# kamenbliznashki/chexpert

Hardware: AMD Instinct MI355X
Metric: images/sec fwd+bwd DenseNet121 320x320 bf16 (per-GPU rate in config.images_per_sec_per_gpu) (higher is better)
Workload: dtype bf16; 1 GPU; densenet121 bf16 1xMI355X 320x320 bs=256 per GPU, U-Ones labels (BASELINE configs[1]); 14 classes; random-init weights, synthetic uint8 X-rays; per_gpu_batch=256, global_batch=256, parallelism=dp1, rccl_ranks=1, capture_failed=0, launch=hipGraph replay

## Files before the change

chexpert_amd/csrc/common.h:

```cpp
#pragma once
#include <hip/hip_runtime.h>
#include <stdint.h>
#include <stdio.h>
#include "../../include/chexpert_hip.h"

#ifdef CX_DIAG
#include <stdlib.h>
static inline int cx_diag_int(const char* name, int dflt) {
  const char* e = getenv(name);
  return e ? atoi(e) : dflt;
}
static inline bool cx_diag_set(const char* name) { return getenv(name) != nullptr; }
#else
static inline int cx_diag_int(const char*, int dflt) { return dflt; }
static inline bool cx_diag_set(const char*) { return false; }
#endif

typedef __bf16 bf16;
typedef __attribute__((ext_vector_type(8))) __bf16 bf16x8;
typedef __attribute__((ext_vector_type(4))) __bf16 bf16x4;
typedef __attribute__((ext_vector_type(4))) short s16x4;
typedef __attribute__((ext_vector_type(16))) float f32x16;
typedef __attribute__((ext_vector_type(4))) float f32x4;

// ... 245 lines not shown
extern thread_local int cx_tl_slab_floats_v;
static inline float* dw_slab(float* scratch, long long scratch_floats, long long splits, long long total) {
  const bool ok = scratch && splits * total <= scratch_floats && splits * total < (1ll << 31);
  cx_tl_slab_floats_v = ok ? (int)(splits * total) : 0;
  return ok ? scratch : nullptr;
}
int cx_dw_reduce(float* dw, const float* slab, size_t total, int splits, hipStream_t st);
int cx_dw_reduce_ld(float* dw, const float* slab, size_t total, int splits, int cols, int dw_ld, hipStream_t st);

static inline int stat_rows_check(const CxConv& p, int rows) {
  if (!p.stat_det || !p.stat_sum) return 0;
  if (rows > p.stat_replicas || p.stat_rstride < p.N) return CX_ESTATROWS;
  cx_tl_stat_rows = rows;
  return 0;
}
```

chexpert_amd/csrc/conv1x1_bwd.hip:

```cpp
#include <cstdlib>
#include <type_traits>
#include "common.h"

namespace {

#ifndef CX_PW_NT
#define CX_PW_NT 7
#endif
constexpr int PW_NT = CX_PW_NT;
constexpr int KD = 128;
constexpr int BM = 128;
constexpr int PITCH = KD * 2 + 16;
constexpr int A_BYTES = BM * PITCH;
constexpr int XH_PITCH = 64;
constexpr int XH_BYTES = BM * XH_PITCH;

template <int CTRL>
__device__ __forceinline__ float dpp_add(float v) {
  return v + __int_as_float(__builtin_amdgcn_update_dpp(0, __float_as_int(v), CTRL, 0xF, 0xF, true));
}
__device__ __forceinline__ float half_sum(float v) {
  v = dpp_add<0xB1>(v);
  v = dpp_add<0x4E>(v);
  v = dpp_add<0x141>(v);
// ... 219 lines not shown
    wg_stat_end<NT / 64>(scratch, BC, tid, NT, p.stat_sum, p.stat_sq, p.stat_det, p.stat_det ? split : (int)blockIdx.x, p.stat_replicas,
                         p.stat_rstride, c0, p.N);
  }
}

constexpr int BM2 = 64;
#ifdef CX_PW_FWD_ORDER
#define TILE_OF(mt) (mt)
#else
#define TILE_OF(mt) (m_tiles - 1 - (mt))
#endif
constexpr int A2_BYTES = BM2 * PITCH;
constexpr int XH2_BYTES = BM2 * XH_PITCH;
typedef uint32_t pw_u32x4 __attribute__((ext_vector_type(4)));
__device__ __forceinline__ uint4 as_u4(const pw_u32x4 v) { return make_uint4(v[0], v[1], v[2], v[3]); }

template <int PRO, bool ACC>
__global__ __launch_bounds__(512, 1) void pw_bwd2_kernel(const CxConv p, float* __restrict__ dw, const int M, const int c_tiles,
                                                         const int tiles_per_split, float* __restrict__ slab, const int dw_ld) {
  constexpr int BC = 128, NT = 512;
  constexpr int W_BYTES = BC * PITCH;
  constexpr int COEF_BYTES = (5 * BC + 3 * KD) * 4;
  extern __shared__ __attribute__((aligned(16))) char smem[];
  float* ecoef = reinterpret_cast<float*>(smem);
  char* Wt = smem + COEF_BYTES;
  char* At = Wt + W_BYTES;
  char* Xh = At + 2 * A2_BYTES;
  char* Xt = Xh + 2 * 4 * XH2_BYTES;
  char* Ot = Xt + A2_BYTES;

  const int tid = threadIdx.x, lane = tid & 63, wave = tid >> 6;
  const int lrow = lane & 31, lh = lane >> 5;
  const int id = xcd_remap(blockIdx.x, gridDim.x);
  const int ct = id % c_tiles, split = id / c_tiles;
  const int c0 = ct * BC;
  const int m_tiles = (M + BM2 - 1) / BM2;
  const int t0 = split * tiles_per_split;
  const int t1 = (t0 + tiles_per_split < m_tiles) ? t0 + tiles_per_split : m_tiles;

  const bf16* __restrict__ X = reinterpret_cast<const bf16*>(p.x);
  const bf16* __restrict__ X2 = reinterpret_cast<const bf16*>(p.x2);
  const bf16* __restrict__ Wp = reinterpret_cast<const bf16*>(p.w);
  const bf16* __restrict__ EX = reinterpret_cast<const bf16*>(p.ex);
  bf16* __restrict__ Y = reinterpret_cast<bf16*>(p.y);

  if (tid < BC) {
    const int n = c0 + tid;
    const bool ok = n < p.N;
    ecoef[tid] = ok ? p.e_sc[n] : 0.f;
    ecoef[BC + tid] = ok ? p.e_sh[n] : 0.f;
    ecoef[2 * BC + tid] = ok ? p.e_mu[n] : 0.f;
    ecoef[3 * BC + tid] = ok ? p.e_r[n] : 0.f;
    ecoef[4 * BC + tid] = ok ? p.e_scale[n] : 0.f;
  }
  const int q = tid & 15, r0 = tid >> 4;
#pragma unroll
  for (int i = 0; i < BC / 32; ++i) {
    const int n = c0 + r0 + 32 * i;
    const uint4 v = *reinterpret_cast<const uint4*>(Wp + (size_t)(n < p.N ? n : 0) * KD + q * 8);
    *reinterpret_cast<uint4*>(Wt + (r0 + 32 * i) * PITCH + q * 16) = n < p.N ? v : make_uint4(0, 0, 0, 0);
  }
  if (PRO == CX_PRO_AFFINE2 && tid < KD) {
    ecoef[5 * BC + tid] = p.pa[tid];
    ecoef[5 * BC + KD + tid] = p.pb[tid];
    ecoef[5 * BC + 2 * KD + tid] = p.pc[tid];
  }
  const float* aco = ecoef + 5 * BC + q * 8;

  const int pw = wave & 1, cq = wave >> 1;
  const int wn = wave & 3, wc0 = (wave >> 2) * 2;
  f32x16 accw[2];
#pragma unroll
  for (int i = 0; i < 2; ++i)
#pragma unroll
    for (int r = 0; r < 16; ++r) accw[i][r] = 0.f;
  float s1[2][8], s2[2][8];
#pragma unroll
  for (int cc = 0; cc < 2; ++cc)
#pragma unroll
    for (int e = 0; e < 8; ++e) s1[cc][e] = s2[cc][e] = 0.f;

// ... 14 lines not shown
        else os[i] = *reinterpret_cast<const pw_u32x4*>(Y + (size_t)mmc * p.ldy + qcl);
      } else os[i] = pw_u32x4{0u, 0u, 0u, 0u};
    }
  };
  auto request_dz = [&](int mt) __attribute__((always_inline)) {
#pragma unroll
    for (int i = 0; i < 2; ++i) {
      const int mm = TILE_OF(mt) * BM2 + r0 + 32 * i;
      const int mmc = mm < M ? mm : M - 1;
      ru[i] = *reinterpret_cast<const pw_u32x4*>(X + (size_t)mmc * p.ldx + q * 8);
      if (PRO == CX_PRO_AFFINE2) rv[i] = *reinterpret_cast<const pw_u32x4*>(X2 + (size_t)mmc * p.ldx2 + q * 8);
    }
  };
  request_dz(t0);
  request_rmw(t0, xsA, osA);
  request_rmw(t0 + 1 < t1 ? t0 + 1 : t0, xsB, osB);
  __syncthreads();

  auto tile = [&](const int mt, auto SelC, pw_u32x4 (&xs)[2], pw_u32x4 (&os)[2]) __attribute__((always_inline)) {
    constexpr int SEL = decltype(SelC)::value;
    const int m0 = TILE_OF(mt) * BM2;
    const bool tvalid = mt < t1;
    char* Ab_ = At + SEL * A2_BYTES;
    char* Xb_ = Xh + SEL * (4 * XH2_BYTES);
    char* Ob_ = Ot + SEL * A2_BYTES;
#pragma unroll
    for (int i = 0; i < 2; ++i) {
      const int row = r0 + 32 * i;
      U128 o;
      if (PRO == CX_PRO_NONE) o.u = as_u4(ru[i]);
      else o.u = cx_affine2_8(as_u4(ru[i]), as_u4(rv[i]), aco, aco + KD, aco + 2 * KD);
      const unsigned keep = (tvalid && m0 + row < M) ? 0xffffffffu : 0u;
      o.u.x &= keep; o.u.y &= keep; o.u.z &= keep; o.u.w &= keep;
      *reinterpret_cast<uint4*>(Ab_ + row * PITCH + q * 16) = o.u;
      *reinterpret_cast<pw_u32x4*>(Xt + row * PITCH + q * 16) = xs[i];
      *reinterpret_cast<pw_u32x4*>(Ob_ + row * PITCH + q * 16) = os[i];
    }
    __syncthreads();
    request_dz(mt + 1 < t1 ? mt + 1 : t1 - 1);
    f32x16 accd;
#pragma unroll
    for (int r = 0; r < 16; ++r) accd[r] = 0.f;
    {
      const char* Ab = Ab_ + (pw * 32 + lrow) * PITCH + lh * 16;
      const char* Wb = Wt + (cq * 32 + lrow) * PITCH + lh * 16;
#pragma unroll
      for (int kk = 0; kk < KD / 16; ++kk) {
        const bf16x8 af = *reinterpret_cast<const bf16x8*>(Ab + kk * 32);
        const bf16x8 wf = *reinterpret_cast<const bf16x8*>(Wb + kk * 32);
        accd = __builtin_amdgcn_mfma_f32_32x32x16_bf16(wf, af, accd, 0, 0, 0);
      }
    }
    const int m = m0 + pw * 32 + lrow;
    const bool pok = tvalid && m < M;
#pragma unroll
    for (int cc = 0; cc < 2; ++cc) {
      const int cl = cq * 32 + 8 * (2 * cc + lh);
// ... 33 lines not shown
    for (int kk = 0; kk < BM2 / 16; ++kk) {
      const bf16x8 af = tr_frag(Ab_, PITCH, kk * 16, wn * 32, lane);
#pragma unroll
      for (int i = 0; i < 2; ++i) {
        const bf16x8 bfr = tr_frag(Xb_ + (wc0 + i) * XH2_BYTES, XH_PITCH, kk * 16, 0, lane);
        accw[i] = __builtin_amdgcn_mfma_f32_32x32x16_bf16(af, bfr, accw[i], 0, 0, 0);
      }
    }
  };

  const int n_pairs = (t1 - t0 + 1) >> 1;
  for (int pr_ = 0; pr_ < n_pairs; ++pr_) {
    tile(t0 + 2 * pr_, std::integral_constant<int, 0>{}, xsA, osA);
    tile(t0 + 2 * pr_ + 1, std::integral_constant<int, 1>{}, xsB, osB);
  }

#pragma unroll
  for (int i = 0; i < 2; ++i) {
    const int c = c0 + (wc0 + i) * 32 + lrow;
    if (c < p.N) {
#pragma unroll
      for (int r = 0; r < 16; ++r) {
        const int n = wn * 32 + (r & 3) + 8 * (r >> 2) + 4 * lh;
        dw_out(dw, slab, (size_t)KD * p.N, split, slab ? (size_t)n * p.N + c : (size_t)n * dw_ld + c, accw[i][r]);
      }
    }
  }
  {
    __syncthreads();
    float* scratch = reinterpret_cast<float*>(At);
    wg_stat_begin<8>(scratch, BC, tid, NT);
    float t1v = 0.f, t2v = 0.f;
#pragma unroll
    for (int cc = 0; cc < 2; ++cc)
#pragma unroll
      for (int e = 0; e < 8; ++e) {
        const float a = half_sum(s1[cc][e]);
        const float b = half_sum(s2[cc][e]);
        if (lrow == 8 * cc + e) { t1v = a; t2v = b; }
      }
    if (lrow < 16) {
      const int cl = cq * 32 + 8 * (2 * (lrow >> 3) + lh) + (lrow & 7);
      wg_stat_put(scratch, BC, wave, cl, t1v, ecoef[3 * BC + cl] * (t2v - ecoef[2 * BC + cl] * t1v));
    }
    wg_stat_end<8>(scratch, BC, tid, NT, p.stat_sum, p.stat_sq, p.stat_det, p.stat_det ? split : (int)blockIdx.x, p.stat_replicas,
                   p.stat_rstride, c0, p.N);
  }
}

struct PairLayer {
  const bf16* x;
  const bf16* x2;
  const bf16* w;
  const float *pa, *pb, *pc;
  const float *e_sc, *e_sh, *e_mu, *e_r, *e_scale;
  float *stat_sum, *stat_sq;
  float* dw;
  float* slab;
  int ldx, ldx2, dw_ld, stat_rstride;
};

template <bool ACC>
// ... 403 lines not shown
  if (const int e = pair_check(*pa)) return e;
  if (const int e = pair_check(*pb)) return e;
  const CxConv &a = *pa, &b = *pb;
  if (a.ex != b.ex || a.y != b.y || a.N != b.N || a.B != b.B || a.H != b.H || a.W != b.W || a.ldex != b.ldex || a.ldy != b.ldy ||
      a.accumulate != b.accumulate || a.stat_det != b.stat_det || a.stat_replicas != b.stat_replicas ||
      dw_ld_a < a.N || a.stat_sum == b.stat_sum)
    return CX_EINVAL;
  hipStream_t st = as_stream(stream);
  return a.accumulate ? launch_bwd2p<true>(a, b, dw_a, dw_ld_a, dw_b, scratch, scratch_floats, st)
                      : launch_bwd2p<false>(a, b, dw_a, dw_ld_a, dw_b, scratch, scratch_floats, st);
}

extern "C" int cx_conv1x1_dgrad_wgrad(const CxConv* pp, float* dw, void* stream) {
  return cx_conv1x1_dgrad_wgrad_ws(pp, dw, nullptr, 0, stream);
}
```

chexpert_amd/csrc/conv1x1_fwdk.hip:

```cpp
#include <cstdlib>
#include "common.h"

namespace {

constexpr int BM = 128, BN = 128;
constexpr int WAVES_N = 2, TM = 2, TN = 2;
constexpr int EPITCH = BN + 4;

template <int BK, int PRO>
__global__ __launch_bounds__(256, 2) void pw_fwdk_kernel(const CxConv p, const int M) {
  constexpr int PITCH = BK * 2 + 16;
  constexpr int CPR = BK / 8;
  constexpr int RPP = 256 / CPR;
  constexpr int NL = 128 / RPP;
  constexpr int A_BYTES = BM * PITCH;
  extern __shared__ __attribute__((aligned(16))) char smem[];
  float* coef = reinterpret_cast<float*>(smem);
  char* At = smem + 2 * p.K * 4;
  char* Bt = At + A_BYTES;
  const int tid = threadIdx.x, lane = tid & 63, wave = tid >> 6;
  const int wm = wave / WAVES_N, wn = wave % WAVES_N;
  const int mt = xcd_remap(blockIdx.x, gridDim.x);
  const bf16* __restrict__ X = reinterpret_cast<const bf16*>(p.x);
  const bf16* __restrict__ Wp = reinterpret_cast<const bf16*>(p.w);
  bf16* __restrict__ Y = reinterpret_cast<bf16*>(p.y);

  if (PRO == CX_PRO_AFFINE_RELU)
    for (int i = tid; i < p.K; i += 256) { coef[i] = p.pa[i]; coef[p.K + i] = p.pb[i]; }

  const int q = tid % CPR, r0 = tid / CPR;
  const int nsteps = (p.K + BK - 1) / BK;
  uint4 ra[NL], rw[NL];
  bool kok = true;
  auto issue_loads = [&](int s) __attribute__((always_inline)) {
    const int c = s * BK + q * 8;
    kok = c < p.K;
    const int cc = kok ? c : 0;
#pragma unroll
    for (int i = 0; i < NL; ++i) {
      const int row = r0 + RPP * i;
      const int m = mt * BM + row;
      const int mc = m < M ? m : M - 1;
      ra[i] = *reinterpret_cast<const uint4*>(X + (size_t)mc * p.ldx + cc);
// ... 15 lines not shown
      }
      *reinterpret_cast<uint4*>(At + row * PITCH + q * 16) = o.u;
      *reinterpret_cast<uint4*>(Bt + row * PITCH + q * 16) = kok ? rw[i] : make_uint4(0, 0, 0, 0);
    }
  };

  f32x16 acc[TM][TN];
#pragma unroll
  for (int i = 0; i < TM; ++i)
#pragma unroll
    for (int j = 0; j < TN; ++j)
#pragma unroll
      for (int r = 0; r < 16; ++r) acc[i][j][r] = 0.f;

  issue_loads(0);
  __syncthreads();
  const int lrow = lane & 31, lh = lane >> 5;
  for (int s = 0; s < nsteps; ++s) {
    write_stage(s);
    __syncthreads();
    if (s + 1 < nsteps) issue_loads(s + 1);
#pragma unroll
    for (int kk = 0; kk < BK / 16; ++kk) {
      bf16x8 af[TM], bfr[TN];
#pragma unroll
      for (int i = 0; i < TM; ++i) af[i] = *reinterpret_cast<const bf16x8*>(At + ((wm * TM + i) * 32 + lrow) * PITCH + kk * 32 + lh * 16);
#pragma unroll
      for (int j = 0; j < TN; ++j) bfr[j] = *reinterpret_cast<const bf16x8*>(Bt + ((wn * TN + j) * 32 + lrow) * PITCH + kk * 32 + lh * 16);
#pragma unroll
      for (int i = 0; i < TM; ++i)
#pragma unroll
        for (int j = 0; j < TN; ++j) acc[i][j] = __builtin_amdgcn_mfma_f32_32x32x16_bf16(af[i], bfr[j], acc[i][j], 0, 0, 0);
    }
    __syncthreads();
  }

  constexpr int ECPR = BN / 8, ERPP = 256 / ECPR, NPASS = 64 / ERPP;
  const int cq = tid % ECPR, rr = tid / ECPR;
  float* etile = reinterpret_cast<float*>(At);
  float s1[8], s2[8];
#pragma unroll
  for (int j = 0; j < 8; ++j) s1[j] = s2[j] = 0.f;
  const bool want_stats = p.stat_sum != nullptr;
#pragma unroll
  for (int half = 0; half < 2; ++half) {
    if (wm == half) {
#pragma unroll
      for (int i = 0; i < TM; ++i)
#pragma unroll
        for (int j = 0; j < TN; ++j)
#pragma unroll
// ... 20 lines not shown
            w4[j] = cx_packbf(v[2 * j], v[2 * j + 1]);
            const float rl = cx_bf_lo(w4[j]), rh = cx_bf_hi(w4[j]);
            s1[2 * j] += rl;
            s1[2 * j + 1] += rh;
            s2[2 * j] += rl * rl;
            s2[2 * j + 1] += rh * rh;
          }
          o.u = make_uint4(w4[0], w4[1], w4[2], w4[3]);
        }
        *reinterpret_cast<uint4*>(Y + (size_t)m * p.ldy + cq * 8) = o.u;
      }
    }
    __syncthreads();
  }
  if (want_stats) {
#pragma unroll
    for (int j = 0; j < 8; ++j) {
#pragma unroll
      for (int d = ECPR; d < 64; d <<= 1) {
        s1[j] += __shfl_xor(s1[j], d);
        s2[j] += __shfl_xor(s2[j], d);
      }
    }
    float* scratch = reinterpret_cast<float*>(At);
    wg_stat_begin<4>(scratch, BN, tid, 256);
    if (lane < ECPR) {
#pragma unroll
      for (int j = 0; j < 8; ++j) wg_stat_put(scratch, BN, wave, cq * 8 + j, s1[j], s2[j]);
    }
    wg_stat_end<4>(scratch, BN, tid, 256, p.stat_sum, p.stat_sq, p.stat_det, (int)blockIdx.x, p.stat_replicas, p.stat_rstride, 0, p.N);
  }
}

template <int PRO, int D>
__global__ __launch_bounds__(256, 2) void pw_fwdp_kernel(const CxConv p, const int M) {
  constexpr int BK = 64;
  constexpr int PITCH = BK * 2 + 16;
  constexpr int CPR = BK / 8;
  constexpr int RPP = 256 / CPR;
  constexpr int NL = 128 / RPP;
  constexpr int A_BYTES = BM * PITCH;
  extern __shared__ __attribute__((aligned(16))) char smem[];
  float* coef = reinterpret_cast<float*>(smem);
  char* At = smem + 2 * p.K * 4;
  char* Bt = At + A_BYTES;
  const int tid = threadIdx.x, lane = tid & 63, wave = tid >> 6;
  const int wm = wave / WAVES_N, wn = wave % WAVES_N;
  const int mt = xcd_remap(blockIdx.x, gridDim.x);
  const bf16* __restrict__ X = reinterpret_cast<const bf16*>(p.x);
  const bf16* __restrict__ Wp = reinterpret_cast<const bf16*>(p.w);
  bf16* __restrict__ Y = reinterpret_cast<bf16*>(p.y);
  if (PRO == CX_PRO_AFFINE_RELU)
    for (int i = tid; i < p.K; i += 256) { coef[i] = p.pa[i]; coef[p.K + i] = p.pb[i]; }
  const int q = tid % CPR, r0 = tid / CPR;
  const int nsteps = (p.K + BK - 1) / BK;
  const bf16* xr[NL];
  const bf16* wr[NL];
#pragma unroll
  for (int i = 0; i < NL; ++i) {
    const int row = r0 + RPP * i;
    const int m = mt * BM + row;
    xr[i] = X + (size_t)(m < M ? m : M - 1) * p.ldx + q * 8;
    wr[i] = Wp + (size_t)row * p.K + q * 8;
  }
  uint4 ra[D][NL], rw[D][NL];
  auto issue = [&](uint4 (&a)[NL], uint4 (&w)[NL], int s) __attribute__((always_inline)) {
    const int sc = s < nsteps ? s : nsteps - 1;
    int c = sc * BK;
// ... 17 lines not shown
        o.u = a[i];
      } else {
        o.u = cx_affine_relu8(a[i], coef + c0, coef + p.K + c0);
      }
      *reinterpret_cast<uint4*>(At + row * PITCH + q * 16) = o.u;
      *reinterpret_cast<uint4*>(Bt + row * PITCH + q * 16) = kok ? w[i] : make_uint4(0, 0, 0, 0);
    }
  };
  f32x16 acc[TM][TN];
#pragma unroll
  for (int i = 0; i < TM; ++i)
#pragma unroll
    for (int j = 0; j < TN; ++j)
#pragma unroll
      for (int r = 0; r < 16; ++r) acc[i][j][r] = 0.f;
#pragma unroll
  for (int d = 0; d < D; ++d) issue(ra[d], rw[d], d);
  __syncthreads();
  const int lrow = lane & 31, lh = lane >> 5;
  for (int s0 = 0; s0 < nsteps; s0 += D) {
#pragma unroll
    for (int d = 0; d < D; ++d) {
      const int s = s0 + d;
      if (s < nsteps) {
        stage(ra[d], rw[d], s);
        __syncthreads();
        issue(ra[d], rw[d], s + D);
#pragma unroll
        for (int kk = 0; kk < BK / 16; ++kk) {
          bf16x8 af[TM], bfr[TN];
#pragma unroll
          for (int i = 0; i < TM; ++i) af[i] = *reinterpret_cast<const bf16x8*>(At + ((wm * TM + i) * 32 + lrow) * PITCH + kk * 32 + lh * 16);
#pragma unroll
          for (int j = 0; j < TN; ++j) bfr[j] = *reinterpret_cast<const bf16x8*>(Bt + ((wn * TN + j) * 32 + lrow) * PITCH + kk * 32 + lh * 16);
#pragma unroll
          for (int i = 0; i < TM; ++i)
#pragma unroll
            for (int j = 0; j < TN; ++j) acc[i][j] = __builtin_amdgcn_mfma_f32_32x32x16_bf16(af[i], bfr[j], acc[i][j], 0, 0, 0);
        }
        __syncthreads();
      }
    }
  }
  constexpr int ECPR = BN / 8, ERPP = 256 / ECPR, NPASS = 64 / ERPP;
  const int cq = tid % ECPR, rr = tid / ECPR;
  float* etile = reinterpret_cast<float*>(At);
  float s1[8], s2[8];
#pragma unroll
  for (int j = 0; j < 8; ++j) s1[j] = s2[j] = 0.f;
  const bool want_stats = p.stat_sum != nullptr;
#pragma unroll
  for (int half = 0; half < 2; ++half) {
    if (wm == half) {
#pragma unroll
      for (int i = 0; i < TM; ++i)
#pragma unroll
        for (int j = 0; j < TN; ++j)
#pragma unroll
// ... 20 lines not shown
            w4[j] = cx_packbf(v[2 * j], v[2 * j + 1]);
            const float rl = cx_bf_lo(w4[j]), rh = cx_bf_hi(w4[j]);
            s1[2 * j] += rl;
            s1[2 * j + 1] += rh;
            s2[2 * j] += rl * rl;
            s2[2 * j + 1] += rh * rh;
          }
          o.u = make_uint4(w4[0], w4[1], w4[2], w4[3]);
        }
        *reinterpret_cast<uint4*>(Y + (size_t)m * p.ldy + cq * 8) = o.u;
      }
    }
    __syncthreads();
  }
  if (want_stats) {
#pragma unroll
    for (int j = 0; j < 8; ++j) {
#pragma unroll
      for (int d = ECPR; d < 64; d <<= 1) {
        s1[j] += __shfl_xor(s1[j], d);
        s2[j] += __shfl_xor(s2[j], d);
      }
    }
    float* scratch = reinterpret_cast<float*>(At);
    wg_stat_begin<4>(scratch, BN, tid, 256);
    if (lane < ECPR) {
#pragma unroll
      for (int j = 0; j < 8; ++j) wg_stat_put(scratch, BN, wave, cq * 8 + j, s1[j], s2[j]);
    }
    wg_stat_end<4>(scratch, BN, tid, 256, p.stat_sum, p.stat_sq, p.stat_det, (int)blockIdx.x, p.stat_replicas, p.stat_rstride, 0, p.N);
  }
}

template <int PRO, int D>
int launch_fwdp(const CxConv& p, hipStream_t st) {
  const long long M = (long long)p.B * p.Ho * p.Wo;
  const int m_tiles = (int)((M + BM - 1) / BM);
  const size_t stage = (size_t)2 * BM * (64 * 2 + 16);
  const size_t epi = (size_t)64 * EPITCH * 4;
  const size_t smem = (size_t)2 * p.K * 4 + (stage > epi ? stage : epi) + 2 * BN * 4;
  static bool attr = false;
  if (!attr) {
    (void)hipFuncSetAttribute(reinterpret_cast<const void*>(&pw_fwdp_kernel<PRO, D>), hipFuncAttributeMaxDynamicSharedMemorySize, 80 * 1024);
    attr = true;
  }
  if (smem > 80 * 1024) return CX_ESHAPE;
// ... 28 lines not shown
  *handled = false;
  if (p.mode != CX_MODE_CONV || p.kh != 1 || p.kw != 1 || p.stride != 1 || p.pad != 0 || p.tstride > 1) return 0;
  if (p.epilogue != CX_EPI_STORE || p.accumulate || p.N != 128 || p.K <= 256 || p.K > 1280) return 0;
  if (p.prologue != CX_PRO_AFFINE_RELU && p.prologue != CX_PRO_NONE) return 0;
  if ((long long)p.B * p.Ho * p.Wo > 200000) return 0;
  *handled = true;
  static const int pipe = cx_diag_int("CX_FWDK_PIPE", 2);
  if (pipe == 2 && p.K % 32 == 0 && p.K >= 512)
    return p.prologue == CX_PRO_AFFINE_RELU ? launch_fwdp<CX_PRO_AFFINE_RELU, 2>(p, st) : launch_fwdp<CX_PRO_NONE, 2>(p, st);
  if (pipe == 3 && p.K % 32 == 0 && p.K >= 192)
    return p.prologue == CX_PRO_AFFINE_RELU ? launch_fwdp<CX_PRO_AFFINE_RELU, 3>(p, st) : launch_fwdp<CX_PRO_NONE, 3>(p, st);
  if (pipe == 4 && p.K % 32 == 0 && p.K >= 256)
    return p.prologue == CX_PRO_AFFINE_RELU ? launch_fwdp<CX_PRO_AFFINE_RELU, 4>(p, st) : launch_fwdp<CX_PRO_NONE, 4>(p, st);
  return p.prologue == CX_PRO_AFFINE_RELU ? launch_fwdk<128, CX_PRO_AFFINE_RELU>(p, st) : launch_fwdk<128, CX_PRO_NONE>(p, st);
}
```

chexpert_amd/csrc/conv3x3_ring.hip:

```cpp
#include <cstdlib>
#include <type_traits>
#include "common.h"

namespace {

constexpr int XP = 272;
constexpr int NT = 512;
constexpr int W_ROWS = 9 * 32;
constexpr int W_BYTES = W_ROWS * XP;
constexpr int RING_PX_MAX = (160 * 1024 - W_BYTES - 1024 - 256) / XP;

struct RingGeo {
  int B, H, W, P, R, Q;
  int Wt, ntx;
  int spi;
  int steps_per_wg;
  unsigned mP;
  unsigned mSpi;
  int ntx_shift;
};

__device__ __forceinline__ int wrapq(int v, int q) { return v >= q ? v - q : v; }
__device__ __forceinline__ int div_spi(const RingGeo& g, int v) { return g.spi == 1 ? v : (int)__umulhi((unsigned)v, g.mSpi); }

template <int CTRL>
__device__ __forceinline__ float dpp_get(float v) { return __int_as_float(__builtin_amdgcn_update_dpp(0, __float_as_int(v), CTRL, 0xF, 0xF, true)); }
template <int XOR>
__device__ __forceinline__ float swz_xor(float v) { return __int_as_float(__builtin_amdgcn_ds_swizzle(__float_as_int(v), (XOR << 10) | 0x1F)); }
__device__ __forceinline__ float half_sum16(const float (&v)[16], int lane) {
  const bool b0 = lane & 1, b1 = lane & 2, b2 = lane & 4, b3 = lane & 8;
  float a[8], b[4], c[2];
#pragma unroll
  for (int k = 0; k < 8; ++k) a[k] = (b0 ? v[2 * k + 1] : v[2 * k]) + dpp_get<0xB1>(b0 ? v[2 * k] : v[2 * k + 1]);
#pragma unroll
  for (int k = 0; k < 4; ++k) b[k] = (b1 ? a[2 * k + 1] : a[2 * k]) + dpp_get<0x4E>(b1 ? a[2 * k] : a[2 * k + 1]);
#pragma unroll
  for (int k = 0; k < 2; ++k) c[k] = (b2 ? b[2 * k + 1] : b[2 * k]) + swz_xor<4>(b2 ? b[2 * k] : b[2 * k + 1]);
  const float d = (b3 ? c[1] : c[0]) + swz_xor<8>(b3 ? c[0] : c[1]);
  return d + swz_xor<16>(d);
}

#ifdef CX_RING_STAMPS
__device__ unsigned long long ring_stamps[1024 * 8];
__device__ unsigned long long ring_fwd_stamps[1024 * 8];
__device__ __forceinline__ unsigned long long rstamp() {
  unsigned long long t;
  __builtin_amdgcn_sched_barrier(0);
  asm volatile("s_memtime %0\n\ts_waitcnt lgkmcnt(0)" : "=s"(t)::"memory");
  __builtin_amdgcn_sched_barrier(0);
  return t;
}
#define RSTAMP(i) { const unsigned long long t_ = rstamp(); st_acc[i] += t_ - st_prev; st_prev = t_; }
__device__ unsigned long long ring_pro_stamps[1024 * 8];
__device__ unsigned long long ring_fwd_pro_stamps[1024 * 8];
#define PSTAMP_BEGIN unsigned long long ps_acc[3] = {0, 0, 0}; const unsigned long long ps_rt0 = __builtin_amdgcn_s_memrealtime(), ps_t0 = rstamp(); \
  unsigned long long ps_prev = ps_t0; bool ps_first = true;
#define PSTAMP(i) { const unsigned long long t_ = rstamp(); ps_acc[i] = t_ - ps_prev; ps_prev = t_; }
#define PSTAMP_FIRST_MFMA if (ps_first) { PSTAMP(1) ps_first = false; }
#define PSTAMP_MARK ps_prev = rstamp();
#define PSTAMP_END(arr) { PSTAMP(2) const unsigned long long rt_ = __builtin_amdgcn_s_memrealtime(); \
  if (threadIdx.x == 0 && blockIdx.x < 1024) { for (int i = 0; i < 3; ++i) arr[blockIdx.x * 8 + i] = ps_acc[i]; \
    arr[blockIdx.x * 8 + 3] = ps_prev - ps_t0; arr[blockIdx.x * 8 + 4] = rt_ - ps_rt0; } }
#else
#define RSTAMP(i)
#define PSTAMP_BEGIN
#define PSTAMP(i)
#define PSTAMP_FIRST_MFMA
#define PSTAMP_MARK
#define PSTAMP_END(arr)
#endif
template <int NCH, int DEPTH>
__global__ __launch_bounds__(NT, 1) void conv3x3_ring_fwd_kernel(const bf16* __restrict__ x, int ldx, const float* __restrict__ sc,
                                                                const float* __restrict__ sh, const bf16* __restrict__ wpk,
                                                                bf16* __restrict__ y, int ldy, float* stat_sum, float* stat_sq,
                                                                int stat_replicas, int stat_rstride, int stat_det, const RingGeo g) {
  extern __shared__ __attribute__((aligned(16))) char smem[];
  float* coef = reinterpret_cast<float*>(smem);
  char* wl = smem + 1024 + 256;
  char* ring = wl + W_BYTES;
  const int tid = threadIdx.x, lane = tid & 63, wave = tid >> 6;
  const int lrow = lane & 31, lh = lane >> 5;
  const int P = g.P, R = g.R, Q = g.Q, W = g.W, H = g.H, Wt = g.Wt, ntx = g.ntx;
  PSTAMP_BEGIN

// ... 934 lines not shown
```

scratch/trace_step.py:

```python
import csv, re, sys
rows = [r for r in csv.DictReader(open(sys.argv[1]))]
rows.sort(key=lambda r: int(r['Start_Timestamp']))
name = lambda r: re.sub(r'\(.*', '', r['Kernel_Name'].replace('void (anonymous namespace)::', '').replace('(anonymous namespace)::', ''))[:48]
idx = [i for i, r in enumerate(rows) if 'adam' in r['Kernel_Name']]
pairs = [(x, y) for x, y in zip(idx, idx[1:]) if y - x > 200]
which = int(sys.argv[2]) if len(sys.argv) > 2 else len(pairs) // 2
a, b = pairs[which]
step = rows[a + 1:b + 1]
t0 = int(step[0]['Start_Timestamp'])
last_end = t0
print("# %d steps; step %d: %d kernels, %.3f ms" % (len(pairs), which, len(step), (int(step[-1]['End_Timestamp']) - t0) / 1e6))
for r in step:
    s, e = int(r['Start_Timestamp']), int(r['End_Timestamp'])
    print("%9.1f %8.1f %7.1f q%-3s %s  g=%s wg=%s" % ((s - t0) / 1e3, (e - s) / 1e3, (s - last_end) / 1e3, r.get('Queue_Id', '?')[-3:], name(r),
                                                   r.get('Grid_Size', r.get('Grid_Size_X', '?')), r.get('Workgroup_Size', r.get('Workgroup_Size_X', '?'))))
    last_end = max(last_end, e)
```

Baseline: 9665 images/sec.

## Overlap pointwise conv prologue loads and shorten BN-stat wave reductions

In the 1x1 conv forward and backward kernels, the weight tile and BN coefficient loads are now issued into registers alongside the first activation tile loads. They are stored to LDS only after a scheduling barrier, so their global latency overlaps instead of serializing before the main loop. The per-channel statistic reductions change too: the backward kernel uses a transposed DPP/swizzle half-sum that reduces 16 values at once, and the forward kernels use permlane16/32 swaps instead of shuffle-xor trees. Optional timestamp instrumentation is added, compiled out by default. The cost is extra register pressure from holding the prefetched values.

```diff
diff --git a/chexpert_amd/csrc/common.h b/chexpert_amd/csrc/common.h
--- a/chexpert_amd/csrc/common.h
+++ b/chexpert_amd/csrc/common.h
@@ -283,3 +283,45 @@
   cx_tl_stat_rows = rows;
   return 0;
 }
+
+template <int CTRL>
+__device__ __forceinline__ float dpp_get(float v) { return __int_as_float(__builtin_amdgcn_update_dpp(0, __float_as_int(v), CTRL, 0xF, 0xF, true)); }
+template <int XOR>
+__device__ __forceinline__ float swz_xor(float v) { return __int_as_float(__builtin_amdgcn_ds_swizzle(__float_as_int(v), (XOR << 10) | 0x1F)); }
+__device__ __forceinline__ float half_sum16(const float (&v)[16], int lane) {
+  const bool b0 = lane & 1, b1 = lane & 2, b2 = lane & 4, b3 = lane & 8;
+  float a[8], b[4], c[2];
+#pragma unroll
+  for (int k = 0; k < 8; ++k) a[k] = (b0 ? v[2 * k + 1] : v[2 * k]) + dpp_get<0xB1>(b0 ? v[2 * k] : v[2 * k + 1]);
+#pragma unroll
+  for (int k = 0; k < 4; ++k) b[k] = (b1 ? a[2 * k + 1] : a[2 * k]) + dpp_get<0x4E>(b1 ? a[2 * k] : a[2 * k + 1]);
+#pragma unroll
+  for (int k = 0; k < 2; ++k) c[k] = (b2 ? b[2 * k + 1] : b[2 * k]) + swz_xor<4>(b2 ? b[2 * k] : b[2 * k + 1]);
+  const float d = (b3 ? c[1] : c[0]) + swz_xor<8>(b3 ? c[0] : c[1]);
+  return d + swz_xor<16>(d);
+}
+
+
+#if defined(CX_RING_STAMPS) || defined(CX_PW_STAMPS)
+__device__ __forceinline__ unsigned long long rstamp() {
+  unsigned long long t;
+  __builtin_amdgcn_sched_barrier(0);
+  asm volatile("s_memtime %0\n\ts_waitcnt lgkmcnt(0)" : "=s"(t)::"memory");
+  __builtin_amdgcn_sched_barrier(0);
+  return t;
+}
+#define PSTAMP_BEGIN unsigned long long ps_acc[3] = {0, 0, 0}; const unsigned long long ps_rt0 = __builtin_amdgcn_s_memrealtime(), ps_t0 = rstamp(); \
+  unsigned long long ps_prev = ps_t0; bool ps_first = true;
+#define PSTAMP(i) { const unsigned long long t_ = rstamp(); ps_acc[i] = t_ - ps_prev; ps_prev = t_; }
+#define PSTAMP_FIRST_MFMA if (ps_first) { PSTAMP(1) ps_first = false; }
+#define PSTAMP_MARK ps_prev = rstamp();
+#define PSTAMP_END(arr) { PSTAMP(2) const unsigned long long rt_ = __builtin_amdgcn_s_memrealtime(); \
+  if (threadIdx.x == 0 && blockIdx.x < 1024) { for (int i = 0; i < 3; ++i) arr[blockIdx.x * 8 + i] = ps_acc[i]; \
+    arr[blockIdx.x * 8 + 3] = ps_prev - ps_t0; arr[blockIdx.x * 8 + 4] = rt_ - ps_rt0; } }
+#else
+#define PSTAMP_BEGIN
+#define PSTAMP(i)
+#define PSTAMP_FIRST_MFMA
+#define PSTAMP_MARK
+#define PSTAMP_END(arr)
+#endif
diff --git a/chexpert_amd/csrc/conv1x1_bwd.hip b/chexpert_amd/csrc/conv1x1_bwd.hip
--- a/chexpert_amd/csrc/conv1x1_bwd.hip
+++ b/chexpert_amd/csrc/conv1x1_bwd.hip
@@ -257,6 +257,9 @@
 constexpr int XH2_BYTES = BM2 * XH_PITCH;
 typedef uint32_t pw_u32x4 __attribute__((ext_vector_type(4)));
 __device__ __forceinline__ uint4 as_u4(const pw_u32x4 v) { return make_uint4(v[0], v[1], v[2], v[3]); }
+#ifdef CX_PW_STAMPS
+__device__ unsigned long long pw_bwd_pro_stamps[1024 * 8];
+#endif
 
 template <int PRO, bool ACC>
 __global__ __launch_bounds__(512, 1) void pw_bwd2_kernel(const CxConv p, float* __restrict__ dw, const int M, const int c_tiles,
@@ -286,28 +289,9 @@
   const bf16* __restrict__ Wp = reinterpret_cast<const bf16*>(p.w);
   const bf16* __restrict__ EX = reinterpret_cast<const bf16*>(p.ex);
   bf16* __restrict__ Y = reinterpret_cast<bf16*>(p.y);
-
-  if (tid < BC) {
-    const int n = c0 + tid;
-    const bool ok = n < p.N;
-    ecoef[tid] = ok ? p.e_sc[n] : 0.f;
-    ecoef[BC + tid] = ok ? p.e_sh[n] : 0.f;
-    ecoef[2 * BC + tid] = ok ? p.e_mu[n] : 0.f;
-    ecoef[3 * BC + tid] = ok ? p.e_r[n] : 0.f;
-    ecoef[4 * BC + tid] = ok ? p.e_scale[n] : 0.f;
-  }
+  PSTAMP_BEGIN
+
   const int q = tid & 15, r0 = tid >> 4;
-#pragma unroll
-  for (int i = 0; i < BC / 32; ++i) {
-    const int n = c0 + r0 + 32 * i;
-    const uint4 v = *reinterpret_cast<const uint4*>(Wp + (size_t)(n < p.N ? n : 0) * KD + q * 8);
-    *reinterpret_cast<uint4*>(Wt + (r0 + 32 * i) * PITCH + q * 16) = n < p.N ? v : make_uint4(0, 0, 0, 0);
-  }
-  if (PRO == CX_PRO_AFFINE2 && tid < KD) {
-    ecoef[5 * BC + tid] = p.pa[tid];
-    ecoef[5 * BC + KD + tid] = p.pb[tid];
-    ecoef[5 * BC + 2 * KD + tid] = p.pc[tid];
-  }
   const float* aco = ecoef + 5 * BC + q * 8;
 
   const int pw = wave & 1, cq = wave >> 1;
@@ -352,8 +336,45 @@
   };
   request_dz(t0);
   request_rmw(t0, xsA, osA);
-  request_rmw(t0 + 1 < t1 ? t0 + 1 : t0, xsB, osB);
+  {
+    pw_u32x4 wv[BC / 32];
+#pragma unroll
+    for (int i = 0; i < BC / 32; ++i) {
+      const int n = c0 + r0 + 32 * i;
+      wv[i] = *reinterpret_cast<const pw_u32x4*>(Wp + (size_t)(n < p.N ? n : 0) * KD + q * 8);
+    }
+    const int en = c0 + (tid & (BC - 1));
+    const bool eok = en < p.N;
+    const int enc = eok ? en : p.N - 1;
+    const float v_sc = p.e_sc[enc], v_sh = p.e_sh[enc], v_mu = p.e_mu[enc], v_r = p.e_r[enc], v_scale = p.e_scale[enc];
+    float v_a = 0.f, v_b = 0.f, v_c = 0.f;
+    if (PRO == CX_PRO_AFFINE2) {
+      v_a = p.pa[tid & (KD - 1)];
+      v_b = p.pb[tid & (KD - 1)];
+      v_c = p.pc[tid & (KD - 1)];
+    }
+    request_rmw(t0 + 1 < t1 ? t0 + 1 : t0, xsB, osB);
+    __builtin_amdgcn_sched_barrier(0);
+#pragma unroll
+    for (int i = 0; i < BC / 32; ++i) {
+      const int n = c0 + r0 + 32 * i;
+      *reinterpret_cast<pw_u32x4*>(Wt + (r0 + 32 * i) * PITCH + q * 16) = n < p.N ? wv[i] : pw_u32x4{0u, 0u, 0u, 0u};
+    }
+    if (tid < BC) {
+      ecoef[tid] = eok ? v_sc : 0.f;
+      ecoef[BC + tid] = eok ? v_sh : 0.f;
+      ecoef[2 * BC + tid] = eok ? v_mu : 0.f;
+      ecoef[3 * BC + tid] = eok ? v_r : 0.f;
+      ecoef[4 * BC + tid] = eok ? v_scale : 0.f;
+    }
+    if (PRO == CX_PRO_AFFINE2 && tid < KD) {
+      ecoef[5 * BC + tid] = v_a;
+      ecoef[5 * BC + KD + tid] = v_b;
+      ecoef[5 * BC + 2 * KD + tid] = v_c;
+    }
+  }
   __syncthreads();
+  PSTAMP(0)
 
   auto tile = [&](const int mt, auto SelC, pw_u32x4 (&xs)[2], pw_u32x4 (&os)[2]) __attribute__((always_inline)) {
     constexpr int SEL = decltype(SelC)::value;
@@ -379,6 +400,7 @@
     f32x16 accd;
 #pragma unroll
     for (int r = 0; r < 16; ++r) accd[r] = 0.f;
+    PSTAMP_FIRST_MFMA
     {
       const char* Ab = Ab_ + (pw * 32 + lrow) * PITCH + lh * 16;
       const char* Wb = Wt + (cq * 32 + lrow) * PITCH + lh * 16;
@@ -442,6 +464,7 @@
     tile(t0 + 2 * pr_, std::integral_constant<int, 0>{}, xsA, osA);
     tile(t0 + 2 * pr_ + 1, std::integral_constant<int, 1>{}, xsB, osB);
   }
+  PSTAMP_MARK
 
 #pragma unroll
   for (int i = 0; i < 2; ++i) {
@@ -455,25 +478,28 @@
     }
   }
   {
+    float f1[16], f2[16];
+#pragma unroll
+    for (int cc = 0; cc < 2; ++cc)
+#pragma unroll
+      for (int e = 0; e < 8; ++e) { f1[8 * cc + e] = s1[cc][e]; f2[8 * cc + e] = s2[cc][e]; }
+    const float t1v = half_sum16(f1, lane), t2v = half_sum16(f2, lane);
     __syncthreads();
     float* scratch = reinterpret_cast<float*>(At);
-    wg_stat_begin<8>(scratch, BC, tid, NT);
-    float t1v = 0.f, t2v = 0.f;
-#pragma unroll
-    for (int cc = 0; cc < 2; ++cc)
-#pragma unroll
-      for (int e = 0; e < 8; ++e) {
-        const float a = half_sum(s1[cc][e]);
-        const float b = half_sum(s2[cc][e]);
-        if (lrow == 8 * cc + e) { t1v = a; t2v = b; }
-      }
     if (lrow < 16) {
       const int cl = cq * 32 + 8 * (2 * (lrow >> 3) + lh) + (lrow & 7);
-      wg_stat_put(scratch, BC, wave, cl, t1v, ecoef[3 * BC + cl] * (t2v - ecoef[2 * BC + cl] * t1v));
+      scratch[(wave * 2) * BC + cl] = t1v;
+      scratch[(wave * 2 + 1) * BC + cl] = ecoef[3 * BC + cl] * (t2v - ecoef[2 * BC + cl] * t1v);
+#pragma unroll
+      for (int k = 1; k < 4; ++k) {
+        scratch[(wave * 2) * BC + ((cl + 32 * k) & (BC - 1))] = 0.f;
+        scratch[(wave * 2 + 1) * BC + ((cl + 32 * k) & (BC - 1))] = 0.f;
+      }
     }
     wg_stat_end<8>(scratch, BC, tid, NT, p.stat_sum, p.stat_sq, p.stat_det, p.stat_det ? split : (int)blockIdx.x, p.stat_replicas,
                    p.stat_rstride, c0, p.N);
   }
+  PSTAMP_END(pw_bwd_pro_stamps)
 }
 
 struct PairLayer {
@@ -907,3 +933,9 @@
 extern "C" int cx_conv1x1_dgrad_wgrad(const CxConv* pp, float* dw, void* stream) {
   return cx_conv1x1_dgrad_wgrad_ws(pp, dw, nullptr, 0, stream);
 }
+
+#ifdef CX_PW_STAMPS
+extern "C" int dbg_pw_bwd_pro_stamps(unsigned long long* host, int n_words) {
+  return (int)hipMemcpyFromSymbol(host, HIP_SYMBOL(pw_bwd_pro_stamps), (size_t)n_words * 8, 0, hipMemcpyDeviceToHost);
+}
+#endif
diff --git a/chexpert_amd/csrc/conv1x1_fwdk.hip b/chexpert_amd/csrc/conv1x1_fwdk.hip
--- a/chexpert_amd/csrc/conv1x1_fwdk.hip
+++ b/chexpert_amd/csrc/conv1x1_fwdk.hip
@@ -6,6 +6,46 @@
 constexpr int BM = 128, BN = 128;
 constexpr int WAVES_N = 2, TM = 2, TN = 2;
 constexpr int EPITCH = BN + 4;
+
+constexpr int COEF_PER_THREAD = 1280 / 256;
+__device__ __forceinline__ void coef_request(const CxConv& p, int tid, float (&ca)[COEF_PER_THREAD], float (&cb)[COEF_PER_THREAD]) {
+#pragma unroll
+  for (int j = 0; j < COEF_PER_THREAD; ++j) {
+    const int i = tid + 256 * j;
+    const int ic = i < p.K ? i : p.K - 1;
+    ca[j] = p.pa[ic];
+    cb[j] = p.pb[ic];
+  }
+}
+__device__ __forceinline__ void coef_store(float* coef, int K, int tid, const float (&ca)[COEF_PER_THREAD], const float (&cb)[COEF_PER_THREAD]) {
+#pragma unroll
+  for (int j = 0; j < COEF_PER_THREAD; ++j) {
+    const int i = tid + 256 * j;
+    if (i < K) { coef[i] = ca[j]; coef[K + i] = cb[j]; }
+  }
+}
+
+__device__ __forceinline__ void wave_stat_rows(float* scratch, int wave, int lane, const float (&s1)[8], const float (&s2)[8]) {
+  float t[8];
+#pragma unroll
+  for (int j = 0; j < 8; ++j) {
+    const auto sw = __builtin_amdgcn_permlane16_swap(__float_as_uint(s1[j]), __float_as_uint(s2[j]), false, false);
+    t[j] = __uint_as_float(sw[0]) + __uint_as_float(sw[1]);
+  }
+  float4 u;
+  float* uu = reinterpret_cast<float*>(&u);
+#pragma unroll
+  for (int j = 0; j < 4; ++j) {
+    const auto sw = __builtin_amdgcn_permlane32_swap(__float_as_uint(t[j]), __float_as_uint(t[j + 4]), false, false);
+    uu[j] = __uint_as_float(sw[0]) + __uint_as_float(sw[1]);
+  }
+  const int kind = (lane >> 4) & 1, cq = lane & 15, lh = lane >> 5;
+  *reinterpret_cast<float4*>(scratch + (wave * 2 + kind) * BN + cq * 8 + lh * 4) = u;
+}
+
+#ifdef CX_PW_STAMPS
+__device__ unsigned long long pw_fwd_pro_stamps[1024 * 8];
+#endif
 
 template <int BK, int PRO>
 __global__ __launch_bounds__(256, 2) void pw_fwdk_kernel(const CxConv p, const int M) {
@@ -24,9 +64,7 @@
   const bf16* __restrict__ X = reinterpret_cast<const bf16*>(p.x);
   const bf16* __restrict__ Wp = reinterpret_cast<const bf16*>(p.w);
   bf16* __restrict__ Y = reinterpret_cast<bf16*>(p.y);
-
-  if (PRO == CX_PRO_AFFINE_RELU)
-    for (int i = tid; i < p.K; i += 256) { coef[i] = p.pa[i]; coef[p.K + i] = p.pb[i]; }
+  PSTAMP_BEGIN
 
   const int q = tid % CPR, r0 = tid / CPR;
   const int nsteps = (p.K + BK - 1) / BK;
@@ -72,12 +110,20 @@
       for (int r = 0; r < 16; ++r) acc[i][j][r] = 0.f;
 
   issue_loads(0);
+  if (PRO == CX_PRO_AFFINE_RELU) {
+    float ca[COEF_PER_THREAD], cb[COEF_PER_THREAD];
+    coef_request(p, tid, ca, cb);
+    __builtin_amdgcn_sched_barrier(0);
+    coef_store(coef, p.K, tid, ca, cb);
+  }
   __syncthreads();
+  PSTAMP(0)
   const int lrow = lane & 31, lh = lane >> 5;
   for (int s = 0; s < nsteps; ++s) {
     write_stage(s);
     __syncthreads();
     if (s + 1 < nsteps) issue_loads(s + 1);
+    PSTAMP_FIRST_MFMA
 #pragma unroll
     for (int kk = 0; kk < BK / 16; ++kk) {
       bf16x8 af[TM], bfr[TN];
@@ -93,6 +139,7 @@
     __syncthreads();
   }
 
+  PSTAMP_MARK
   constexpr int ECPR = BN / 8, ERPP = 256 / ECPR, NPASS = 64 / ERPP;
   const int cq = tid % ECPR, rr = tid / ECPR;
   float* etile = reinterpret_cast<float*>(At);
@@ -143,22 +190,11 @@
     __syncthreads();
   }
   if (want_stats) {
-#pragma unroll
-    for (int j = 0; j < 8; ++j) {
-#pragma unroll
-      for (int d = ECPR; d < 64; d <<= 1) {
-        s1[j] += __shfl_xor(s1[j], d);
-        s2[j] += __shfl_xor(s2[j], d);
-      }
-    }
     float* scratch = reinterpret_cast<float*>(At);
-    wg_stat_begin<4>(scratch, BN, tid, 256);
-    if (lane < ECPR) {
-#pragma unroll
-      for (int j = 0; j < 8; ++j) wg_stat_put(scratch, BN, wave, cq * 8 + j, s1[j], s2[j]);
-    }
+    wave_stat_rows(scratch, wave, lane, s1, s2);
     wg_stat_end<4>(scratch, BN, tid, 256, p.stat_sum, p.stat_sq, p.stat_det, (int)blockIdx.x, p.stat_replicas, p.stat_rstride, 0, p.N);
   }
+  PSTAMP_END(pw_fwd_pro_stamps)
 }
 
 template <int PRO, int D>
@@ -179,8 +215,7 @@
   const bf16* __restrict__ X = reinterpret_cast<const bf16*>(p.x);
   const bf16* __restrict__ Wp = reinterpret_cast<const bf16*>(p.w);
   bf16* __restrict__ Y = reinterpret_cast<bf16*>(p.y);
-  if (PRO == CX_PRO_AFFINE_RELU)
-    for (int i = tid; i < p.K; i += 256) { coef[i] = p.pa[i]; coef[p.K + i] = p.pb[i]; }
+  PSTAMP_BEGIN
   const int q = tid % CPR, r0 = tid / CPR;
   const int nsteps = (p.K + BK - 1) / BK;
   const bf16* xr[NL];
@@ -228,9 +263,15 @@
     for (int j = 0; j < TN; ++j)
 #pragma unroll
       for (int r = 0; r < 16; ++r) acc[i][j][r] = 0.f;
-#pragma unroll
-  for (int d = 0; d < D; ++d) issue(ra[d], rw[d], d);
+  issue(ra[0], rw[0], 0);
+  float ca[COEF_PER_THREAD], cb[COEF_PER_THREAD];
+  if (PRO == CX_PRO_AFFINE_RELU) coef_request(p, tid, ca, cb);
+#pragma unroll
+  for (int d = 1; d < D; ++d) issue(ra[d], rw[d], d);
+  __builtin_amdgcn_sched_barrier(0);
+  if (PRO == CX_PRO_AFFINE_RELU) coef_store(coef, p.K, tid, ca, cb);
   __syncthreads();
+  PSTAMP(0)
   const int lrow = lane & 31, lh = lane >> 5;
   for (int s0 = 0; s0 < nsteps; s0 += D) {
 #pragma unroll
@@ -240,6 +281,7 @@
         stage(ra[d], rw[d], s);
         __syncthreads();
         issue(ra[d], rw[d], s + D);
+        PSTAMP_FIRST_MFMA
 #pragma unroll
         for (int kk = 0; kk < BK / 16; ++kk) {
           bf16x8 af[TM], bfr[TN];
@@ -256,6 +298,7 @@
       }
     }
   }
+  PSTAMP_MARK
   constexpr int ECPR = BN / 8, ERPP = 256 / ECPR, NPASS = 64 / ERPP;
   const int cq = tid % ECPR, rr = tid / ECPR;
   float* etile = reinterpret_cast<float*>(At);
@@ -306,22 +349,11 @@
     __syncthreads();
   }
   if (want_stats) {
-#pragma unroll
-    for (int j = 0; j < 8; ++j) {
-#pragma unroll
-      for (int d = ECPR; d < 64; d <<= 1) {
-        s1[j] += __shfl_xor(s1[j], d);
-        s2[j] += __shfl_xor(s2[j], d);
-      }
-    }
     float* scratch = reinterpret_cast<float*>(At);
-    wg_stat_begin<4>(scratch, BN, tid, 256);
-    if (lane < ECPR) {
-#pragma unroll
-      for (int j = 0; j < 8; ++j) wg_stat_put(scratch, BN, wave, cq * 8 + j, s1[j], s2[j]);
-    }
+    wave_stat_rows(scratch, wave, lane, s1, s2);
     wg_stat_end<4>(scratch, BN, tid, 256, p.stat_sum, p.stat_sq, p.stat_det, (int)blockIdx.x, p.stat_replicas, p.stat_rstride, 0, p.N);
   }
+  PSTAMP_END(pw_fwd_pro_stamps)
 }
 
 template <int PRO, int D>
@@ -380,3 +412,9 @@
     return p.prologue == CX_PRO_AFFINE_RELU ? launch_fwdp<CX_PRO_AFFINE_RELU, 4>(p, st) : launch_fwdp<CX_PRO_NONE, 4>(p, st);
   return p.prologue == CX_PRO_AFFINE_RELU ? launch_fwdk<128, CX_PRO_AFFINE_RELU>(p, st) : launch_fwdk<128, CX_PRO_NONE>(p, st);
 }
+
+#ifdef CX_PW_STAMPS
+extern "C" int dbg_pw_fwd_pro_stamps(unsigned long long* host, int n_words) {
+  return (int)hipMemcpyFromSymbol(host, HIP_SYMBOL(pw_fwd_pro_stamps), (size_t)n_words * 8, 0, hipMemcpyDeviceToHost);
+}
+#endif
diff --git a/chexpert_amd/csrc/conv3x3_ring.hip b/chexpert_amd/csrc/conv3x3_ring.hip
--- a/chexpert_amd/csrc/conv3x3_ring.hip
+++ b/chexpert_amd/csrc/conv3x3_ring.hip
@@ -23,51 +23,14 @@
 __device__ __forceinline__ int wrapq(int v, int q) { return v >= q ? v - q : v; }
 __device__ __forceinline__ int div_spi(const RingGeo& g, int v) { return g.spi == 1 ? v : (int)__umulhi((unsigned)v, g.mSpi); }
 
-template <int CTRL>
-__device__ __forceinline__ float dpp_get(float v) { return __int_as_float(__builtin_amdgcn_update_dpp(0, __float_as_int(v), CTRL, 0xF, 0xF, true)); }
-template <int XOR>
-__device__ __forceinline__ float swz_xor(float v) { return __int_as_float(__builtin_amdgcn_ds_swizzle(__float_as_int(v), (XOR << 10) | 0x1F)); }
-__device__ __forceinline__ float half_sum16(const float (&v)[16], int lane) {
-  const bool b0 = lane & 1, b1 = lane & 2, b2 = lane & 4, b3 = lane & 8;
-  float a[8], b[4], c[2];
-#pragma unroll
-  for (int k = 0; k < 8; ++k) a[k] = (b0 ? v[2 * k + 1] : v[2 * k]) + dpp_get<0xB1>(b0 ? v[2 * k] : v[2 * k + 1]);
-#pragma unroll
-  for (int k = 0; k < 4; ++k) b[k] = (b1 ? a[2 * k + 1] : a[2 * k]) + dpp_get<0x4E>(b1 ? a[2 * k] : a[2 * k + 1]);
-#pragma unroll
-  for (int k = 0; k < 2; ++k) c[k] = (b2 ? b[2 * k + 1] : b[2 * k]) + swz_xor<4>(b2 ? b[2 * k] : b[2 * k + 1]);
-  const float d = (b3 ? c[1] : c[0]) + swz_xor<8>(b3 ? c[0] : c[1]);
-  return d + swz_xor<16>(d);
-}
-
 #ifdef CX_RING_STAMPS
 __device__ unsigned long long ring_stamps[1024 * 8];
 __device__ unsigned long long ring_fwd_stamps[1024 * 8];
-__device__ __forceinline__ unsigned long long rstamp() {
-  unsigned long long t;
-  __builtin_amdgcn_sched_barrier(0);
-  asm volatile("s_memtime %0\n\ts_waitcnt lgkmcnt(0)" : "=s"(t)::"memory");
-  __builtin_amdgcn_sched_barrier(0);
-  return t;
-}
 #define RSTAMP(i) { const unsigned long long t_ = rstamp(); st_acc[i] += t_ - st_prev; st_prev = t_; }
 __device__ unsigned long long ring_pro_stamps[1024 * 8];
 __device__ unsigned long long ring_fwd_pro_stamps[1024 * 8];
-#define PSTAMP_BEGIN unsigned long long ps_acc[3] = {0, 0, 0}; const unsigned long long ps_rt0 = __builtin_amdgcn_s_memrealtime(), ps_t0 = rstamp(); \
-  unsigned long long ps_prev = ps_t0; bool ps_first = true;
-#define PSTAMP(i) { const unsigned long long t_ = rstamp(); ps_acc[i] = t_ - ps_prev; ps_prev = t_; }
-#define PSTAMP_FIRST_MFMA if (ps_first) { PSTAMP(1) ps_first = false; }
-#define PSTAMP_MARK ps_prev = rstamp();
-#define PSTAMP_END(arr) { PSTAMP(2) const unsigned long long rt_ = __builtin_amdgcn_s_memrealtime(); \
-  if (threadIdx.x == 0 && blockIdx.x < 1024) { for (int i = 0; i < 3; ++i) arr[blockIdx.x * 8 + i] = ps_acc[i]; \
-    arr[blockIdx.x * 8 + 3] = ps_prev - ps_t0; arr[blockIdx.x * 8 + 4] = rt_ - ps_rt0; } }
 #else
 #define RSTAMP(i)
-#define PSTAMP_BEGIN
-#define PSTAMP(i)
-#define PSTAMP_FIRST_MFMA
-#define PSTAMP_MARK
-#define PSTAMP_END(arr)
 #endif
 template <int NCH, int DEPTH>
 __global__ __launch_bounds__(NT, 1) void conv3x3_ring_fwd_kernel(const bf16* __restrict__ x, int ldx, const float* __restrict__ sc,
diff --git a/scratch/stamps_pw.py b/scratch/stamps_pw.py
--- /dev/null
+++ b/scratch/stamps_pw.py
@@ -0,0 +1,48 @@
+import ctypes, shutil, sys, numpy as np, torch
+sys.path.insert(0, '.')
+from chexpert_amd import _lib
+shutil.copy(sys.argv[1] if len(sys.argv) > 1 else "scratch/libstamp_pw.so", _lib.LIB_PATH)
+from chexpert_amd import ops
+dev = torch.device('cuda:0'); bf = torch.bfloat16; B = 256
+ops.set_det_wgrad(True)
+def outside(fn_name, wgs):
+    host = (ctypes.c_ulonglong * (1024 * 8))()
+    getattr(ctypes.CDLL(_lib.LIB_PATH), fn_name)(host, 1024 * 8)
+    a = np.frombuffer(host, dtype=np.uint64).reshape(1024, 8).astype(np.float64)[:min(wgs, 1024)]
+    a = a[a[:, 4] > 0]
+    m = np.median(a, 0)
+    mhz = np.median(a[:, 3] / a[:, 4]) * 100.0
+    return "   clocks per launch at %.0f MHz: setup %.0f (%.2f us), setup -> first MFMA %.0f (%.2f us), entry -> first MFMA %.2f us, last tile -> end %.0f (%.2f us), kernel %.0f (%.2f us)" % (
+        mhz, m[0], m[0] / mhz, m[1], m[1] / mhz, (m[0] + m[1]) / mhz, m[2], m[2] / mhz, m[3], m[3] / mhz)
+def timed(fn):
+    for _ in range(3): fn()
+    torch.cuda.synchronize()
+    e0, e1 = torch.cuda.Event(enable_timing=True), torch.cuda.Event(enable_timing=True)
+    e0.record(); fn(); e1.record(); torch.cuda.synchronize()
+    return e0.elapsed_time(e1) * 1e3
+cap = 4096
+for hw, ctot, cins in ((20, 1024, (512, 1024)), (10, 1024, (512, 1024)), (40, 512, (256,))):
+    M = B * hw * hw
+    buf = (torch.randn(B, hw, hw, ctot, device=dev) * 0.5).to(bf)
+    gbuf = (torch.randn(B, hw, hw, ctot, device=dev) * 0.5).to(bf)
+    y1 = (torch.randn(B, hw, hw, 128, device=dev) * 0.5).to(bf)
+    dz2 = (torch.randn(B, hw, hw, 128, device=dev) * 0.5).to(bf)
+    ones, zeros = torch.ones(1024, device=dev), torch.zeros(1024, device=dev)
+    st = torch.zeros(2, cap * 1024, device=dev)
+    for cin in cins:
+        wf = (torch.randn(128 * cin, device=dev) * 0.05).to(bf)
+        dw = torch.zeros(128, cin, 1, 1, device=dev)
+        if hw <= 20:
+            f = lambda: ops.conv_gemm(buf[..., :cin], wf, y1, N=128, prologue=ops.PRO_AFFINE_RELU, pa=ones, pb=zeros, stat_sum=st[0],
+                                      stat_sq=st[1], stat_det=True, stat_replicas=cap, stat_rstride=128)
+            us = timed(f)
+            print("%dx%d FORWARD K=%d (%s, %.1f us)" % (hw, hw, cin, ops.last_kernel(), us), flush=True)
+            print(outside("dbg_pw_fwd_pro_stamps", (M + 127) // 128), flush=True)
+        d = lambda: ops.conv_gemm(dz2, wf, gbuf[..., :cin], N=cin, prologue=ops.PRO_AFFINE2, x2=y1, pa=ones, pb=zeros, pc=zeros,
+                                  epilogue=ops.EPI_MASK, ex=buf[..., :cin], e_sc=ones, e_sh=zeros, e_mu=zeros, e_r=ones, e_scale=ones,
+                                  stat_sum=st[0], stat_sq=st[1], accumulate=True, stat_det=True, stat_replicas=cap, stat_rstride=1024,
+                                  fused_dw=dw)
+        us = timed(d)
+        print("%dx%d BACKWARD N=%d (%s, %.1f us with the slab sum)" % (hw, hw, cin, ops.last_kernel(), us), flush=True)
+        print(outside("dbg_pw_bwd_pro_stamps", 256), flush=True)
+    del buf, gbuf, y1, dz2
diff --git a/scratch/trace_step.py b/scratch/trace_step.py
--- a/scratch/trace_step.py
+++ b/scratch/trace_step.py
@@ -2,7 +2,7 @@
 rows = [r for r in csv.DictReader(open(sys.argv[1]))]
 rows.sort(key=lambda r: int(r['Start_Timestamp']))
 name = lambda r: re.sub(r'\(.*', '', r['Kernel_Name'].replace('void (anonymous namespace)::', '').replace('(anonymous namespace)::', ''))[:48]
-idx = [i for i, r in enumerate(rows) if 'adam' in r['Kernel_Name']]
+idx = [i for i, r in enumerate(rows) if 'adam' in r['Kernel_Name'].lower()]
 pairs = [(x, y) for x, y in zip(idx, idx[1:]) if y - x > 200]
 which = int(sys.argv[2]) if len(sys.argv) > 2 else len(pairs) // 2
 a, b = pairs[which]
```

Result: no change. 9718 images/sec, median of 6 (+0.6%).
